# MAC-VO/MAC-VO

Measured on AMD Instinct MI355X. Metric: stereo frames/sec at 640x480 (hot path: cost volume + lookup, keypoint selection, covariance, PGO), higher is better.
Workload: dtype f32 via f16x2 (volume: fp32 operands row-scaled by powers of two and split into two fp16 pieces, three products, fp32 accumulate, scales undone exactly) + f32 (lookup/covariance) + f64 (PGO)

## Files before the change

### mac-vo_amd/csrc/frontend_ops.hip

```cpp
#include "common.h"
#include "randperm_dev.h"
#include "kp_draw_dev.h"
#include "match_cov_dev.h"
#include "pose_apply_dev.h"
#include "obs_filter_dev.h"
#include <math.h>

namespace {

__global__ __launch_bounds__(256) void frontend_epilogue_kernel(
    const float* __restrict__ flow, const float* __restrict__ logcov, int cov_is_log, int plane, float bl_fx,
    float bl_fx_sq, float* __restrict__ disparity, float* __restrict__ disparity_cov, float* __restrict__ depth,
    float* __restrict__ depth_cov, uint8_t* __restrict__ bad_mask, float* __restrict__ match_flow,
    float* __restrict__ match_cov) {
    MV_CHAIN_KERNEL_PRIO();
    const size_t lo = (size_t)blockIdx.y * plane;
    flow += 4 * lo; logcov += 4 * lo;
    if (disparity) disparity += lo;
    if (disparity_cov) disparity_cov += lo;
    if (depth) depth += lo;
    if (depth_cov) depth_cov += lo;
    if (bad_mask) bad_mask += lo;
    if (match_flow) match_flow += 2 * lo;
    if (match_cov) match_cov += 3 * lo;
// ... 12 lines not shown
    const size_t lo = (size_t)blockIdx.y * plane;
    flow += 4 * lo;
    if (D || M) logcov += 4 * lo;
    if (disparity) disparity += lo;
    if (D && disparity_cov) disparity_cov += lo;
    if (depth) depth += lo;
    if (D && depth_cov) depth_cov += lo;
    if (bad_mask) bad_mask += lo;
    if (match_flow) match_flow += 2 * lo;
    if (M && match_cov) match_cov += 3 * lo;
    const mvEpiArgs ea{flow, logcov, cov_is_log, bl_fx, bl_fx_sq, disparity, D ? disparity_cov : nullptr, depth, D ? depth_cov : nullptr, match_flow,
                       M ? match_cov : nullptr, bad_mask};
    for (int i = blockIdx.x * blockDim.x + threadIdx.x; i < plane; i += gridDim.x * blockDim.x) mv_epilogue_pixel_partial<D, M>(ea, plane, i);
}

__device__ __forceinline__ void kp_track_one(int n, int u0, int v0, const float* __restrict__ match_flow, const float* __restrict__ match_cov,
                                             const float* __restrict__ depth0, const float* __restrict__ disp0,
                                             const float* __restrict__ sdisp0, const float* __restrict__ sdd0,
                                             const float* __restrict__ depth1, const float* __restrict__ disp1,
                                             const float* __restrict__ sdisp1, const float* __restrict__ sdd1, int H, int W, int edge,
                                             float match_cov_default, float* __restrict__ out_kp0, float* __restrict__ out_kp1,
                                             uint8_t* __restrict__ out_inbound, float* __restrict__ out_vals, size_t vs,
                                             float* __restrict__ out_sigma0, float* __restrict__ out_sigma1) {
    const int plane = H * W;
    const bool ok0 = u0 >= 0 && u0 < W && v0 >= 0 && v0 < H;
    const int i0 = ok0 ? v0 * W + u0 : 0;
    const float u1 = (float)u0 + match_flow[i0];
    const float v1 = (float)v0 + match_flow[plane + i0];
    const bool inb = ok0 && (u1 < (float)(W - edge)) && (u1 > (float)edge) && (v1 < (float)(H - edge)) && (v1 > (float)edge);
    if (out_kp0) { out_kp0[2 * n] = (float)u0; out_kp0[2 * n + 1] = (float)v0; }
    out_kp1[2 * n] = u1;
    out_kp1[2 * n + 1] = v1;
    out_inbound[n] = inb;
    float* o = out_vals + n;
    o[0 * vs] = depth0[i0];
    o[1 * vs] = disp0 ? disp0[i0] : -1.f;
    o[2 * vs] = sdisp0 ? sdisp0[i0] : -1.f;
    o[3 * vs] = sdd0 ? sdd0[i0] : -1.f;
    if (inb) {
        const int i1 = (int)v1 * W + (int)u1;
        o[4 * vs] = depth1[i1];
        o[5 * vs] = disp1 ? disp1[i1] : -1.f;
        o[6 * vs] = sdisp1 ? sdisp1[i1] : -1.f;
        o[7 * vs] = sdd1 ? sdd1[i1] : -1.f;
    } else {
        o[4 * vs] = o[5 * vs] = o[6 * vs] = o[7 * vs] = 0.f;
    }
    const float suu = match_cov ? match_cov[i0] : -1.f;
    const float svv = match_cov ? match_cov[plane + i0] : -1.f;
    const float suv = match_cov ? match_cov[2 * plane + i0] : -1.f;
    o[8 * vs] = suu; o[9 * vs] = svv; o[10 * vs] = suv;
    if (out_sigma1) { out_sigma1[3 * n] = suu; out_sigma1[3 * n + 1] = svv; out_sigma1[3 * n + 2] = suv; }
    if (out_sigma0) { out_sigma0[3 * n] = match_cov_default; out_sigma0[3 * n + 1] = match_cov_default; out_sigma0[3 * n + 2] = 0.f; }
}

struct TrackArgs {
    const float *match_flow, *match_cov, *depth0, *disp0, *sdisp0, *sdd0, *depth1, *disp1, *sdisp1, *sdd1;
    int H, W, edge;
    float match_cov_default;
    float *out_kp0, *out_kp1;
    uint8_t* out_inbound;
    float *out_vals, *out_sigma0, *out_sigma1;
};
__device__ __forceinline__ void track_lane_offsets(TrackArgs& a, int lane, int N) {
    const size_t lp = (size_t)lane * a.H * a.W, ln = (size_t)lane * N;
    a.match_flow += 2 * lp;
    if (a.match_cov) a.match_cov += 3 * lp;
    a.depth0 += lp; a.depth1 += lp;
// ... 31 lines not shown
                                                       int64_t* __restrict__ out_uv, TrackArgs a, float fx, float fy, float cx, float cy,
                                                       float* __restrict__ pos_Tc) {
    const int n = blockIdx.x * blockDim.x + threadIdx.x;
    const int lane = blockIdx.y;
    if (n >= cnt.n[lane]) return;
    cand += (size_t)lane * cand_lane_stride;
    out_uv += 2 * (size_t)lane * cap;
    pos_Tc += 3 * (size_t)lane * cap;
    track_lane_offsets(a, lane, cap);
    const long pi = PERM_IN_ARGS ? (long)pa.idx[n] : (long)perm[(size_t)lane * cap + n];
    const int lin = cand[pi];
    const int u0 = lin % a.W, v0 = lin / a.W;
    out_uv[2 * n + 0] = u0;
    out_uv[2 * n + 1] = v0;
    const size_t vs = (size_t)gridDim.y * cap;
    kp_track_one(n, u0, v0, a.match_flow, a.match_cov, a.depth0, a.disp0, a.sdisp0, a.sdd0, a.depth1, a.disp1, a.sdisp1, a.sdd1, a.H,
                 a.W, a.edge, a.match_cov_default, a.out_kp0, a.out_kp1, a.out_inbound, a.out_vals, vs, a.out_sigma0, a.out_sigma1);
    const float u = (float)u0, v = (float)v0, d = a.out_vals[n];
    pos_Tc[3 * n] = d;
    pos_Tc[3 * n + 1] = ((u - cx) * d) / fx;
    pos_Tc[3 * n + 2] = ((v - cy) * d) / fy;
}

__global__ __launch_bounds__(256) void backproject_kernel(const float* __restrict__ kp_uv,
                                                          const float* __restrict__ depth_vals, int depth_stride,
                                                          float fx, float fy, float cx, float cy,
                                                          const float* __restrict__ pose, int cap, mvLaneCounts cnt,
                                                          size_t depth_lane_stride,
                                                          float* __restrict__ pos_Tc, float* __restrict__ pos_Tw,
                                                          double* __restrict__ rot) {
    const int n = blockIdx.x * blockDim.x + threadIdx.x;
    const int lane = blockIdx.y;
    const int N = cnt.n[lane];
// ... 123 lines not shown
    int32_t out[mvrp::MAX_HEAD];
};
template <int PM, int MODEL = MV_COV_MATCH, bool MODS = false, bool NOMATCH = false>
__global__ __launch_bounds__(256) void backend_front_kernel(const int32_t* __restrict__ cand, size_t cand_lane_stride, const int64_t* __restrict__ perm,
                                                            PermArg pa, int cap, mvLaneCounts cnt, int64_t* out_uv, TrackArgs a, float fx, float fy,
                                                            float cx, float cy, float* pos_Tc, const float* depth_map0, const float* depth_map1,
                                                            double* out_cov0, double* out_cov1, mvMatchCovParams cp, DrawArgs da) {
    __shared__ __attribute__((aligned(16))) char draw_raw[PM == 2 ? sizeof(DrawLds) : PM == 4 ? sizeof(mvkp::Scratch) : 16];
    DrawLds& D = *reinterpret_cast<DrawLds*>(draw_raw);
    const int lane = threadIdx.x & 63;
    const int n = blockIdx.x * 4 + (threadIdx.x >> 6);
    const int set = blockIdx.y, pl = blockIdx.z;
    int N;
    if constexpr (PM == 2) {
        const int64_t n_cand = da.count[(size_t)pl * da.count_stride];
        const bool adv = blockIdx.x == 0 && blockIdx.y == 0;
        N = mv_randperm_head_wg(da.state_in + (size_t)pl * mvrp::MT_STRIDE, adv ? da.state_out + (size_t)pl * mvrp::MT_STRIDE : nullptr, n_cand, da.k,
                                D.out, D.s, D.head);
        __syncthreads();
        if (adv) {
            for (int i = threadIdx.x; i < N; i += 256) da.out_perm[(size_t)pl * cap + i] = D.out[i];
            if (threadIdx.x == 0) { da.out_live[2 * pl] = N; da.out_live[2 * pl + 1] = (int32_t)n_cand; }
        }
    } else if constexpr (PM == 3) {
        if (da.count) {
            const int c = da.count[(size_t)pl * da.count_stride];
            N = c < 0 ? 0 : (c > cap ? cap : c);
        } else {
            N = cnt.n[pl];
        }
        if (da.out_live && blockIdx.x == 0 && blockIdx.y == 0 && threadIdx.x == 0) { da.out_live[2 * pl] = N; da.out_live[2 * pl + 1] = N; }
    } else if constexpr (PM == 4) {
        N = cnt.n[pl];
// ... 12 lines not shown
            u0 = lin % a.W;
            v0 = lin / a.W;
        } else if constexpr (PM == 3) {
            const int64_t* kp = perm + 2 * ((size_t)pl * cap + n);
            u0 = (int)kp[0];
            v0 = (int)kp[1];
        } else if constexpr (PM == 4) {
            mvkp::row_of(reinterpret_cast<mvkp::Scratch*>(draw_raw)->w, da.k, n, a.H, a.W, pa.idx[0], u0, v0);
        } else {
            mvkp::grid_row(mvkp::Grid{pa.idx[0], 0, pa.idx[1], pa.idx[2], pa.idx[3]}, n, u0, v0);
        }
        TrackArgs al = a;
        track_lane_offsets(al, pl, cap);
        const size_t ln = (size_t)pl * cap;
        float u, v, suu, svv, suv;
        if (set == 0) {
            if (lane == 0) {
                if (PM != 3 || out_uv != perm) {
                    out_uv[2 * (ln + n) + 0] = u0;
                    out_uv[2 * (ln + n) + 1] = v0;
                }
                kp_track_one(n, u0, v0, al.match_flow, al.match_cov, al.depth0, al.disp0, al.sdisp0, al.sdd0, al.depth1, al.disp1, al.sdisp1, al.sdd1,
                             al.H, al.W, al.edge, al.match_cov_default, al.out_kp0, al.out_kp1, al.out_inbound, al.out_vals, (size_t)gridDim.z * cap,
                             nullptr, nullptr);
                al.out_sigma0[3 * n + 2] = 0.f;
                const float uf = (float)u0, vf = (float)v0, d = al.out_vals[n];
                float* pt = pos_Tc + 3 * (ln + n);
                pt[0] = d;
                pt[1] = ((uf - cx) * d) / fx;
                pt[2] = ((vf - cy) * d) / fy;
            }
            u = (float)u0; v = (float)v0;
            suu = a.match_cov_default; svv = a.match_cov_default; suv = 0.f;
        } else {
            const int plane = al.H * al.W;
            const bool ok0 = u0 >= 0 && u0 < al.W && v0 >= 0 && v0 < al.H;
            const int i0 = ok0 ? v0 * al.W + u0 : 0;
            u = (float)u0 + al.match_flow[i0];
            v = (float)v0 + al.match_flow[plane + i0];
            if constexpr (NOMATCH) {
                if (lane == 0) { al.out_sigma1[3 * n] = -1.f; al.out_sigma1[3 * n + 1] = -1.f; al.out_sigma1[3 * n + 2] = -1.f; }
                const bool inb = ok0 && (u < (float)(al.W - al.edge)) && (u > (float)al.edge) && (v < (float)(al.H - al.edge)) && (v > (float)al.edge);
                const bool have_var = al.sdd1 != nullptr;
                const float var = have_var && inb ? al.sdd1[(int)v * al.W + (int)u] : 0.f;
                const mvcov::CovSet S1{depth_map1, nullptr, nullptr, nullptr, nullptr, out_cov1, nullptr, nullptr};
                mvcov::match_cov_wave_vals<MODEL, MODS, true>(S1, cp, cap, pl, n, u, v, da.nomatch_c, da.nomatch_c, 0.f, da.cov_mods, a.sdd1, var, have_var);
                return;
            }
            suu = al.match_cov ? al.match_cov[i0] : -1.f;
            svv = al.match_cov ? al.match_cov[plane + i0] : -1.f;
            suv = al.match_cov ? al.match_cov[2 * plane + i0] : -1.f;
            if (lane == 0) al.out_sigma1[3 * n + 2] = suv;
        }
        const mvcov::CovSet S{set ? depth_map1 : depth_map0, nullptr, set ? a.out_sigma1 : a.out_sigma0, nullptr, nullptr, set ? out_cov1 : out_cov0,
                              nullptr, nullptr};
        if constexpr (MODEL == MV_COV_MATCH && !MODS)
            mvcov::match_cov_wave_vals(S, cp, cap, pl, n, u, v, suu, svv, suv);
        else
            mvcov::match_cov_wave_vals<MODEL, MODS>(S, cp, cap, pl, n, u, v, suu, svv, suv, da.cov_mods, set ? a.sdd1 : a.sdd0);
    }
}

template <int PM, typename... Args>
void launch_backend_front(int model, int32_t mods, bool nomatch, float nomatch_c, dim3 grid, hipStream_t st, DrawArgs da, Args... args) {
    const bool m = mods != 0;
    da.cov_mods = mods;
    if constexpr (PM >= 3) if (nomatch) {
        da.nomatch_c = nomatch_c;
        if (model == MV_COV_MATCH && !m)
            hipLaunchKernelGGL((backend_front_kernel<PM, MV_COV_MATCH, false, true>), grid, dim3(256), 0, st, args..., da);
        else if (model == MV_COV_MATCH)
            hipLaunchKernelGGL((backend_front_kernel<PM, MV_COV_MATCH, true, true>), grid, dim3(256), 0, st, args..., da);
        else if (model == MV_COV_GMM && !m)
            hipLaunchKernelGGL((backend_front_kernel<PM, MV_COV_GMM, false, true>), grid, dim3(256), 0, st, args..., da);
// ... 355 lines not shown
```

### mac-vo_amd/csrc/kp_select.hip

```cpp
#include "common.h"
#include <math.h>

namespace {

#ifdef MV_KP_PROFILE
__device__ long long g_kp_stamps[16];
#define KP_STAMP(i) do { if (threadIdx.x == 0) g_kp_stamps[i] = wall_clock64(); } while (0)
#else
#define KP_STAMP(i)
#endif

constexpr int TILE_W = 64;
constexpr int TILE_H = 16;
constexpr int MAX_R = 7;
constexpr unsigned CAND_FLAG = 0x80000000u;

struct KpWs {
    unsigned long long* cand_bits;
    unsigned* rec_idx;
    float* rec_q;
    float* rec_d;
    int* counters;
    size_t lane_bytes;

// ... 341 lines not shown
                for (int j = 0; j < cb; ++j) {
                    const unsigned o = L.lst[j];
                    rank += (o < e) || (o == e && j < i);
                }
                if (rank == k) L.res = e;
            }
            __syncthreads();
            return key_float(L.res);
        }
        lo = nlo;
        hi = nhi;
        __syncthreads();
    }
}

template <int NT, bool FAST, int RPT, int WPT, bool USE_D>
__device__ __forceinline__ void kp_finish_body(const mvKpSelectParams& p, const KpWs& ws, int has_flow, int words_per_row,
                                               int32_t* __restrict__ out_cand, int32_t* __restrict__ out_count,
                                               float* __restrict__ out_stats, int n_rec, MedianLds& L,
                                               unsigned long long* lds_words) {
    constexpr int RD = USE_D ? RPT : 1;
    const int tid = threadIdx.x;
    const int H = p.H, W = p.W;
    const bool mapping = p.mode == MV_KP_MAPPING;
    const bool use_f = (p.mode == MV_KP_NODEPTH) || (p.mode == MV_KP_FULL && has_flow);
    const bool use_d = USE_D && (p.mode == MV_KP_FULL);
    const int n_words = H * words_per_row;

    unsigned kq[RPT], kd[RD], ridx[RPT];
    unsigned long long wreg[WPT];
    KP_STAMP(0);
    if (FAST) {
        const int cap = H * W;
#pragma unroll
        for (int r = 0; r < RPT; ++r) {
            const int i = min(r * NT + tid, cap - 1);
            ridx[r] = mapping ? 0u : ws.rec_idx[i];
            kq[r] = use_f ? __float_as_uint(ws.rec_q[i]) : 0u;
            if (USE_D) kd[r] = use_d ? __float_as_uint(ws.rec_d[i]) : 0u;
        }
#pragma unroll
        for (int j = 0; j < WPT; ++j) {
            const int w = j * NT + tid;
            wreg[j] = w < n_words ? ws.cand_bits[w] : 0ull;
        }
#pragma unroll
        for (int r = 0; r < RPT; ++r) {
            const bool live = r * NT + tid < n_rec;
            ridx[r] = live ? ridx[r] : 0u;
            kq[r] = live ? float_key(__uint_as_float(kq[r])) : NAN_KEY;
            if (USE_D) kd[r] = live ? float_key(__uint_as_float(kd[r])) : NAN_KEY;
        }
    }

    float med_f = NAN, thr_f = INFINITY, med_d = NAN, thr_d = INFINITY;
    KP_STAMP(1);
    if (use_f) {
        med_f = block_nanmedian<NT, FAST, RPT>(ws.rec_q, n_rec, kq, L);
        const float prod = med_f * 1.5f;
        thr_f = (prod < p.max_match_cov) ? prod : p.max_match_cov;
// ... 107 lines not shown
        out_stats[3] = thr_d;
    }
}

template <int NT, int RPT, int WPT, bool USE_D>
__global__ __launch_bounds__(NT) void kp_finish_kernel(mvKpSelectParams p, KpWs ws_all, int has_flow, int words_per_row,
                                                        int32_t* __restrict__ out_cand, int32_t* __restrict__ out_count,
                                                        float* __restrict__ out_stats) {
    __shared__ MedianLds L;
    extern __shared__ unsigned long long lds_words[];
    MV_CHAIN_KERNEL_PRIO();
    const KpWs ws = ws_all.lane(blockIdx.x);
    out_cand += (size_t)blockIdx.x * p.H * p.W;
    out_count += 4 * blockIdx.x;
    out_stats += 4 * blockIdx.x;
    const int n_rec = p.mode == MV_KP_MAPPING ? 0 : ws.counters[0];
    if (n_rec <= RPT * NT && p.H * words_per_row <= WPT * NT)
        kp_finish_body<NT, true, RPT, WPT, USE_D>(p, ws, has_flow, words_per_row, out_cand, out_count, out_stats, n_rec, L,
                                                  lds_words);
    else
        kp_finish_body<NT, false, RPT, WPT, USE_D>(p, ws, has_flow, words_per_row, out_cand, out_count, out_stats, n_rec, L,
                                                   lds_words);
}

template <int NT, int RPT, int WPT, bool USE_D>
static int launch_finish(const mvKpSelectParams& p, const KpWs& ws, int has_flow, int wpr, int32_t* out_cand,
                         int32_t* out_count, float* out_stats, int lanes, hipStream_t s) {
    const size_t dyn = (size_t)WPT * (NT / (WPT > 5 * 1024 / NT ? 8 : 2)) * sizeof(unsigned long long);
    hipLaunchKernelGGL((kp_finish_kernel<NT, RPT, WPT, USE_D>), dim3(lanes), dim3(NT), dyn, s, p, ws, has_flow, wpr, out_cand,
                       out_count, out_stats);
    return MV_OK;
}

__global__ __launch_bounds__(1024) void kp_map_scan_kernel(const unsigned long long* __restrict__ cand_bits, int n_words,
                                                            int* __restrict__ word_off, int32_t* __restrict__ out_count,
                                                            float* __restrict__ out_stats) {
    __shared__ int wave_tot[16];
// ... 189 lines not shown
```

### mac-vo_amd/csrc/match_cov_dev.h

```cpp
#pragma once
#include "common.h"
#include <math.h>

namespace mvcov {

constexpr int MAX_K = 31;
constexpr int MAX_TAPS_PER_LANE = (MAX_K * MAX_K + 63) / 64;

__device__ __forceinline__ float clamp_min_nanprop(float x, float m) { return (x < m) ? m : x; }

struct CovSet {
    const float* depth_map;
    const float* kp_uv;
    float* flow_cov;
    const float* depth_cov;
    const double* rot;
    double* out_cov;
    double* out_cov_rot;
    float* out_stats;
};

__device__ __forceinline__ void apply_modifiers(double c[9], int32_t mods) {
#pragma unroll
    for (int s = 0; s < 4; ++s) {
// ... 25 lines not shown
            for (int j = 0; j < 3; ++j)
                t[3 * i + j] = (R[3 * i] * c[j] + R[3 * i + 1] * c[3 + j]) + R[3 * i + 2] * c[6 + j];
        double* orot = out_cov_rot + (size_t)n * 9;
#pragma unroll
        for (int i = 0; i < 3; ++i)
#pragma unroll
            for (int j = 0; j < 3; ++j)
                orot[3 * i + j] = (t[3 * i] * R[3 * j] + t[3 * i + 1] * R[3 * j + 1]) + t[3 * i + 2] * R[3 * j + 2];
    }
    if (out_stats) {
        out_stats[2 * n] = mu;
        out_stats[2 * n + 1] = var;
    }
}

template <int MODEL = MV_COV_MATCH, bool MODS = false, bool NOMATCH = false>
__device__ __forceinline__ void match_cov_wave_vals(const CovSet& S, const mvMatchCovParams& p, int cap, int pl, int n, float u, float v,
                                                    float suu, float svv, float suv, int32_t mods = 0,
                                                    const float* depth_cov_map_all = nullptr ,
                                                    float var_given = 0.f, bool have_var = false ) {
    const int lane = threadIdx.x & 63;
    const size_t ln = (size_t)pl * cap;
    const float* __restrict__ depth_map = S.depth_map + (size_t)pl * p.H * p.W;
    float* __restrict__ flow_cov = S.flow_cov + 3 * ln;
    const float* __restrict__ depth_cov = S.depth_cov ? S.depth_cov + ln : nullptr;
    const double* __restrict__ rot = S.rot ? S.rot + 9 * pl : nullptr;
    double* __restrict__ out_cov = S.out_cov + 9 * ln;
    double* __restrict__ out_cov_rot = S.out_cov_rot ? S.out_cov_rot + 9 * ln : nullptr;
    float* __restrict__ out_stats = S.out_stats ? S.out_stats + 2 * ln : nullptr;

    if constexpr (MODEL == MV_COV_NONE) {
        if (lane == 0) {
            if constexpr (!NOMATCH) {
                flow_cov[3 * n] = suu;
                flow_cov[3 * n + 1] = svv;
            }
            double c[9] = {1.0, 0.0, 0.0, 0.0, 1.0, 0.0, 0.0, 0.0, 1.0};
            store_cov<MODS>(c, mods, rot, out_cov, out_cov_rot, out_stats, n, __builtin_nanf(""), __builtin_nanf(""));
        }
        return;
    }
    const float* __restrict__ depth_cov_map = MODEL == MV_COV_GMM ? depth_cov_map_all + (size_t)pl * p.H * p.W : nullptr;

    const int iu = (int)u, iv = (int)v;
    if constexpr (!NOMATCH) {
        suu = clamp_min_nanprop(suu, p.min_flow_cov_sq);
        svv = clamp_min_nanprop(svv, p.min_flow_cov_sq);
        if (lane == 0) {
            flow_cov[3 * n] = suu;
            flow_cov[3 * n + 1] = svv;
        }
    }
    bool patch_var;
    if constexpr (NOMATCH) patch_var = !have_var; else patch_var = p.use_patch_var;

    const float det = suu * svv - suv * suv;
    const float m00 = -0.5f * (svv / det), m01 = -0.5f * (-suv / det), m11 = -0.5f * (suu / det);
    const float cnorm = (2.f * 3.14159265358979323846f) * sqrtf(det);

    const int K = p.kernel_size, h = K >> 1, taps = K * K;
    float z[MAX_TAPS_PER_LANE], kv[MAX_TAPS_PER_LANE];
    float zc[MODEL == MV_COV_GMM ? MAX_TAPS_PER_LANE : 1];
    float ksum = 0.f;
#pragma unroll
    for (int r = 0; r < MAX_TAPS_PER_LANE; ++r) {
        const int idx = r * 64 + lane;
        z[r] = 0.f;
        kv[r] = 0.f;
        if constexpr (MODEL == MV_COV_GMM) zc[r] = 0.f;
        if (idx < taps) {
            const int a = idx / K, b = idx - a * K;
            int yy = iv + (a - h), xx = iu + (b - h);
            yy = min(max(yy, 0), p.H - 1);
            xx = min(max(xx, 0), p.W - 1);
            z[r] = depth_map[yy * p.W + xx];
            if constexpr (MODEL == MV_COV_GMM) zc[r] = depth_cov_map[yy * p.W + xx] + z[r] * z[r];
            const float x0 = (float)(a - h), x1 = (float)(b - h);
            const float q = (x0 * m00) * x0 + 2.f * ((x0 * m01) * x1) + (x1 * m11) * x1;
            kv[r] = expf(q) / cnorm;
            ksum += kv[r];
        }
    }
    ksum = wave_sum(ksum);

    float mu = 0.f, var;
    if constexpr (MODEL == MV_COV_GMM) {
        float psum = 0.f;
#pragma unroll
        for (int r = 0; r < MAX_TAPS_PER_LANE; ++r) {
            kv[r] = kv[r] / ksum;
            if (kv[r] < 1e-3f) kv[r] = 0.f;
            psum += kv[r];
        }
        psum = wave_sum(psum);
        float e2 = 0.f;
#pragma unroll
        for (int r = 0; r < MAX_TAPS_PER_LANE; ++r) {
            kv[r] = kv[r] / psum;
            mu += z[r] * kv[r];
            e2 += zc[r] * kv[r];
        }
        mu = wave_sum(mu);
        e2 = wave_sum(e2);
        if constexpr (NOMATCH) var = patch_var ? (e2 - mu * mu) / 2.f : var_given;
// ... 46 lines not shown
                    t[3 * i + j] = (R[3 * i] * c[j] + R[3 * i + 1] * c[3 + j]) + R[3 * i + 2] * c[6 + j];
            double* orot = out_cov_rot + (size_t)n * 9;
#pragma unroll
            for (int i = 0; i < 3; ++i)
#pragma unroll
                for (int j = 0; j < 3; ++j)
                    orot[3 * i + j] = (t[3 * i] * R[3 * j] + t[3 * i + 1] * R[3 * j + 1]) + t[3 * i + 2] * R[3 * j + 2];
        }
        if (out_stats) {
            out_stats[2 * n] = mu;
            out_stats[2 * n + 1] = var;
        }
    }
}


template <int MODEL = MV_COV_MATCH, bool MODS = false>
__device__ __forceinline__ void match_cov_wave(const CovSet& S, const mvMatchCovParams& p, int cap, int pl, int n, int32_t mods = 0,
                                               const float* depth_cov_map = nullptr) {
    const size_t ln = (size_t)pl * cap;
    const float* __restrict__ kp_uv = S.kp_uv + 2 * ln;
    const float* __restrict__ flow_cov = S.flow_cov + 3 * ln;
    match_cov_wave_vals<MODEL, MODS>(S, p, cap, pl, n, kp_uv[2 * n], kp_uv[2 * n + 1], flow_cov[3 * n], flow_cov[3 * n + 1], flow_cov[3 * n + 2],
                                     mods, depth_cov_map);
}

template <int MODEL, bool MODS>
__device__ __forceinline__ void match_cov_wave_nomatch(const CovSet& S, const mvMatchCovParams& p, int cap, int pl, int n, float c, int32_t mods,
                                                       const float* depth_cov_map) {
    const size_t ln = (size_t)pl * cap;
// ... 8 lines not shown
```

### mac-vo_amd/csrc/randperm.hip

```cpp
#include "common.h"
#include "randperm_dev.h"
#include <vector>

int mv_randperm_heads_emulated_state(uint32_t* state, const int64_t* n, int calls, int k, int threads, int64_t* out);

namespace {

__global__ __launch_bounds__(1024) void randperm_head_kernel(uint32_t* __restrict__ state, const int32_t* __restrict__ n_dev, int n_stride, int k, int cap,
                                                             int64_t* __restrict__ out, int32_t* __restrict__ n_sel, int nsel_stride) {
    __shared__ mvrp::Scratch s;
    __shared__ int32_t head[mvrp::NBUCKET];
    const int l = blockIdx.x;
    uint32_t* const st = state + (size_t)l * mvrp::MT_STRIDE;
    const int m = mv_randperm_head_wg(st, st, (int64_t)n_dev[(size_t)l * n_stride], k, out + (size_t)l * cap, s, head);
    if (threadIdx.x == 0) n_sel[(size_t)l * nsel_stride] = m;
}

}

extern "C" int mv_randperm_state_words(void) { return mvrp::MT_STRIDE; }
extern "C" int mv_randperm_max_head(void) { return mvrp::MAX_HEAD; }

extern "C" int mv_mt19937_seed(uint64_t seed, uint32_t* state_host) {
    MV_CHECK_ARG(state_host);
    mvrp::mt_seed((uint32_t)(seed & 0xffffffffull), state_host);
    return MV_OK;
}

extern "C" int mv_randperm_head_lanes(uint32_t* state, const int32_t* n_dev, int n_stride, int lanes, int k, int cap, int64_t* out_perm, int32_t* out_n_sel,
// ... 54 lines not shown
```

### mac-vo_amd/csrc/randperm_dev.h

```cpp
#pragma once
#include <stdint.h>

#if defined(__HIPCC__)
#define MV_RP_FN __host__ __device__ __forceinline__
#else
#define MV_RP_FN inline
#endif

namespace mvrp {

constexpr int MT_N = 624;
constexpr int MT_STRIDE = 640;
constexpr int MAX_HEAD = 512;
constexpr int NBUCKET = 1024;

struct Scratch {
    uint32_t mt[2][MT_N];
    int32_t t[MAX_HEAD], nxt[MAX_HEAD], ptr[MAX_HEAD], hit[MAX_HEAD];
};

MV_RP_FN uint32_t mt_f(uint32_t a, uint32_t b) {
    const uint32_t y = (a & 0x80000000u) | (b & 0x7fffffffu);
    return (y >> 1) ^ ((b & 1u) ? 0x9908b0dfu : 0u);
}
// ... 84 lines not shown
    while (s.ptr[i] >= 0) i = s.ptr[i];
    return i;
}

template <typename T>
MV_RP_FN void phase_emit(const Scratch& s, const Plan& pl, T* out, int tid, int nt) {
    for (int i = tid; i < pl.m; i += nt) {
        const int32_t h = s.hit[i];
        out[i] = (T)(h == -2 ? root_of(s, i) : (h >= 0 ? root_of(s, h) : s.t[i]));
    }
}

}

#if defined(__HIPCC__)
template <typename T>
__device__ __forceinline__ int mv_randperm_head_wg(const uint32_t* __restrict__ state_in, uint32_t* state_out, int64_t n, int k, T* out, mvrp::Scratch& s,
                                                   int32_t* head) {
    using namespace mvrp;
    const int tid = threadIdx.x, nt = blockDim.x;
    const Plan pl = plan_of(n, k);
    phase_clear(head, tid, nt);
    if (pl.advance > 0 || state_out) {
        for (int i = tid; i < MT_N; i += nt) s.mt[0][i] = state_in[i];
        int pos = (int)state_in[MT_N];
        __syncthreads();
        int cur = 0;
        int64_t produced = 0;
        const int64_t total = state_out ? pl.advance : (int64_t)pl.swaps;
        int64_t rem = total;
        while (rem > 0) {
            if (pos == MT_N) {
                phase_step(s.mt[cur], s.mt[cur ^ 1], tid, nt);
                __syncthreads();
                cur ^= 1;
                pos = 0;
            }
            const int take = (int)(rem < MT_N - pos ? rem : MT_N - pos);
            if (produced < pl.swaps) phase_draws(s.mt[cur], pos, take, produced, pl, s.t, tid, nt);
            pos += take;
// ... 1 lines not shown
            rem -= take;
        }
        if (state_out) {
            for (int i = tid; i < MT_N; i += nt) state_out[i] = s.mt[cur][i];
            if (tid == 0) state_out[MT_N] = (uint32_t)pos;
        }
    }
    __syncthreads();
    phase_insert(s, head, pl, tid, nt);
    __syncthreads();
    phase_link(s, head, pl, tid, nt);
    __syncthreads();
    phase_emit(s, pl, out, tid, nt);
    return pl.m;
}
#endif
```

Baseline: 7291.

## Hoist global loads ahead of dependent work in front and select kernels

Splits keypoint tracking into separate load, load-dependent and store phases so the tracker lane's gathers can be issued alongside the covariance window loads in the fused backend front kernel. The randperm state load is hoisted into registers before the draw, and the kp_finish preload of records and candidate bits is moved out of the body. The aim is to hide global-memory latency in small latency-bound kernels, at the cost of more live registers and possible occupancy pressure. A standalone timing probe script is also added.

```diff
diff --git a/mac-vo_amd/csrc/frontend_ops.hip b/mac-vo_amd/csrc/frontend_ops.hip
--- a/mac-vo_amd/csrc/frontend_ops.hip
+++ b/mac-vo_amd/csrc/frontend_ops.hip
@@ -50,44 +50,84 @@
     for (int i = blockIdx.x * blockDim.x + threadIdx.x; i < plane; i += gridDim.x * blockDim.x) mv_epilogue_pixel_partial<D, M>(ea, plane, i);
 }
 
-__device__ __forceinline__ void kp_track_one(int n, int u0, int v0, const float* __restrict__ match_flow, const float* __restrict__ match_cov,
-                                             const float* __restrict__ depth0, const float* __restrict__ disp0,
-                                             const float* __restrict__ sdisp0, const float* __restrict__ sdd0,
-                                             const float* __restrict__ depth1, const float* __restrict__ disp1,
-                                             const float* __restrict__ sdisp1, const float* __restrict__ sdd1, int H, int W, int edge,
-                                             float match_cov_default, float* __restrict__ out_kp0, float* __restrict__ out_kp1,
-                                             uint8_t* __restrict__ out_inbound, float* __restrict__ out_vals, size_t vs,
-                                             float* __restrict__ out_sigma0, float* __restrict__ out_sigma1) {
+struct KpTrackAt0 {
+    bool ok0;
+    float fu, fv, d0, p0, sp0, sd0, suu, svv, suv;
+};
+struct KpTrackAt1 {
+    float u1, v1;
+    bool inb;
+    float d1, p1, sp1, sd1;
+};
+__device__ __forceinline__ KpTrackAt0 kp_track_load0(int u0, int v0, const float* __restrict__ match_flow, const float* __restrict__ match_cov,
+                                                     const float* __restrict__ depth0, const float* __restrict__ disp0,
+                                                     const float* __restrict__ sdisp0, const float* __restrict__ sdd0, int H, int W) {
     const int plane = H * W;
-    const bool ok0 = u0 >= 0 && u0 < W && v0 >= 0 && v0 < H;
-    const int i0 = ok0 ? v0 * W + u0 : 0;
-    const float u1 = (float)u0 + match_flow[i0];
-    const float v1 = (float)v0 + match_flow[plane + i0];
-    const bool inb = ok0 && (u1 < (float)(W - edge)) && (u1 > (float)edge) && (v1 < (float)(H - edge)) && (v1 > (float)edge);
+    KpTrackAt0 t;
+    t.ok0 = u0 >= 0 && u0 < W && v0 >= 0 && v0 < H;
+    const int i0 = t.ok0 ? v0 * W + u0 : 0;
+    t.fu = match_flow[i0];
+    t.fv = match_flow[plane + i0];
+    t.d0 = depth0[i0];
+    t.p0 = disp0 ? disp0[i0] : -1.f;
+    t.sp0 = sdisp0 ? sdisp0[i0] : -1.f;
+    t.sd0 = sdd0 ? sdd0[i0] : -1.f;
+    t.suu = match_cov ? match_cov[i0] : -1.f;
+    t.svv = match_cov ? match_cov[plane + i0] : -1.f;
+    t.suv = match_cov ? match_cov[2 * plane + i0] : -1.f;
+    return t;
+}
+__device__ __forceinline__ KpTrackAt1 kp_track_load1(int u0, int v0, const KpTrackAt0& t0, const float* __restrict__ depth1,
+                                                     const float* __restrict__ disp1, const float* __restrict__ sdisp1,
+                                                     const float* __restrict__ sdd1, int H, int W, int edge) {
+    KpTrackAt1 t;
+    t.u1 = (float)u0 + t0.fu;
+    t.v1 = (float)v0 + t0.fv;
+    t.inb = t0.ok0 && (t.u1 < (float)(W - edge)) && (t.u1 > (float)edge) && (t.v1 < (float)(H - edge)) && (t.v1 > (float)edge);
+    if (t.inb) {
+        const int i1 = (int)t.v1 * W + (int)t.u1;
+        t.d1 = depth1[i1];
+        t.p1 = disp1 ? disp1[i1] : -1.f;
+        t.sp1 = sdisp1 ? sdisp1[i1] : -1.f;
+        t.sd1 = sdd1 ? sdd1[i1] : -1.f;
+    } else {
+        t.d1 = t.p1 = t.sp1 = t.sd1 = 0.f;
+    }
+    return t;
+}
+__device__ __forceinline__ void kp_track_store(int n, int u0, int v0, const KpTrackAt0& t0, const KpTrackAt1& t1, float match_cov_default,
+                                               float* __restrict__ out_kp0, float* __restrict__ out_kp1, uint8_t* __restrict__ out_inbound,
+                                               float* __restrict__ out_vals, size_t vs, float* __restrict__ out_sigma0,
+                                               float* __restrict__ out_sigma1) {
     if (out_kp0) { out_kp0[2 * n] = (float)u0; out_kp0[2 * n + 1] = (float)v0; }
-    out_kp1[2 * n] = u1;
-    out_kp1[2 * n + 1] = v1;
-    out_inbound[n] = inb;
+    out_kp1[2 * n] = t1.u1;
+    out_kp1[2 * n + 1] = t1.v1;
+    out_inbound[n] = t1.inb;
     float* o = out_vals + n;
-    o[0 * vs] = depth0[i0];
-    o[1 * vs] = disp0 ? disp0[i0] : -1.f;
-    o[2 * vs] = sdisp0 ? sdisp0[i0] : -1.f;
-    o[3 * vs] = sdd0 ? sdd0[i0] : -1.f;
-    if (inb) {
-        const int i1 = (int)v1 * W + (int)u1;
-        o[4 * vs] = depth1[i1];
-        o[5 * vs] = disp1 ? disp1[i1] : -1.f;
-        o[6 * vs] = sdisp1 ? sdisp1[i1] : -1.f;
-        o[7 * vs] = sdd1 ? sdd1[i1] : -1.f;
-    } else {
-        o[4 * vs] = o[5 * vs] = o[6 * vs] = o[7 * vs] = 0.f;
-    }
-    const float suu = match_cov ? match_cov[i0] : -1.f;
-    const float svv = match_cov ? match_cov[plane + i0] : -1.f;
-    const float suv = match_cov ? match_cov[2 * plane + i0] : -1.f;
-    o[8 * vs] = suu; o[9 * vs] = svv; o[10 * vs] = suv;
-    if (out_sigma1) { out_sigma1[3 * n] = suu; out_sigma1[3 * n + 1] = svv; out_sigma1[3 * n + 2] = suv; }
+    o[0 * vs] = t0.d0;
+    o[1 * vs] = t0.p0;
+    o[2 * vs] = t0.sp0;
+    o[3 * vs] = t0.sd0;
+    o[4 * vs] = t1.d1;
+    o[5 * vs] = t1.p1;
+    o[6 * vs] = t1.sp1;
+    o[7 * vs] = t1.sd1;
+    o[8 * vs] = t0.suu; o[9 * vs] = t0.svv; o[10 * vs] = t0.suv;
+    if (out_sigma1) { out_sigma1[3 * n] = t0.suu; out_sigma1[3 * n + 1] = t0.svv; out_sigma1[3 * n + 2] = t0.suv; }
     if (out_sigma0) { out_sigma0[3 * n] = match_cov_default; out_sigma0[3 * n + 1] = match_cov_default; out_sigma0[3 * n + 2] = 0.f; }
+}
+__device__ __forceinline__ float kp_track_one(int n, int u0, int v0, const float* __restrict__ match_flow, const float* __restrict__ match_cov,
+                                              const float* __restrict__ depth0, const float* __restrict__ disp0,
+                                              const float* __restrict__ sdisp0, const float* __restrict__ sdd0,
+                                              const float* __restrict__ depth1, const float* __restrict__ disp1,
+                                              const float* __restrict__ sdisp1, const float* __restrict__ sdd1, int H, int W, int edge,
+                                              float match_cov_default, float* __restrict__ out_kp0, float* __restrict__ out_kp1,
+                                              uint8_t* __restrict__ out_inbound, float* __restrict__ out_vals, size_t vs,
+                                              float* __restrict__ out_sigma0, float* __restrict__ out_sigma1) {
+    const KpTrackAt0 t0 = kp_track_load0(u0, v0, match_flow, match_cov, depth0, disp0, sdisp0, sdd0, H, W);
+    const KpTrackAt1 t1 = kp_track_load1(u0, v0, t0, depth1, disp1, sdisp1, sdd1, H, W, edge);
+    kp_track_store(n, u0, v0, t0, t1, match_cov_default, out_kp0, out_kp1, out_inbound, out_vals, vs, out_sigma0, out_sigma1);
+    return t0.d0;
 }
 
 struct TrackArgs {
@@ -149,9 +189,9 @@
     out_uv[2 * n + 0] = u0;
     out_uv[2 * n + 1] = v0;
     const size_t vs = (size_t)gridDim.y * cap;
-    kp_track_one(n, u0, v0, a.match_flow, a.match_cov, a.depth0, a.disp0, a.sdisp0, a.sdd0, a.depth1, a.disp1, a.sdisp1, a.sdd1, a.H,
-                 a.W, a.edge, a.match_cov_default, a.out_kp0, a.out_kp1, a.out_inbound, a.out_vals, vs, a.out_sigma0, a.out_sigma1);
-    const float u = (float)u0, v = (float)v0, d = a.out_vals[n];
+    const float d = kp_track_one(n, u0, v0, a.match_flow, a.match_cov, a.depth0, a.disp0, a.sdisp0, a.sdd0, a.depth1, a.disp1, a.sdisp1, a.sdd1, a.H,
+                                 a.W, a.edge, a.match_cov_default, a.out_kp0, a.out_kp1, a.out_inbound, a.out_vals, vs, a.out_sigma0, a.out_sigma1);
+    const float u = (float)u0, v = (float)v0;
     pos_Tc[3 * n] = d;
     pos_Tc[3 * n + 1] = ((u - cx) * d) / fx;
     pos_Tc[3 * n + 2] = ((v - cy) * d) / fy;
@@ -305,9 +345,9 @@
     int N;
     if constexpr (PM == 2) {
         const int64_t n_cand = da.count[(size_t)pl * da.count_stride];
+        const mvRandpermStateRegs<256> st = mv_randperm_state_load<256>(da.state_in + (size_t)pl * mvrp::MT_STRIDE);
         const bool adv = blockIdx.x == 0 && blockIdx.y == 0;
-        N = mv_randperm_head_wg(da.state_in + (size_t)pl * mvrp::MT_STRIDE, adv ? da.state_out + (size_t)pl * mvrp::MT_STRIDE : nullptr, n_cand, da.k,
-                                D.out, D.s, D.head);
+        N = mv_randperm_head_draw<256>(st, adv ? da.state_out + (size_t)pl * mvrp::MT_STRIDE : nullptr, n_cand, da.k, D.out, D.s, D.head);
         __syncthreads();
         if (adv) {
             for (int i = threadIdx.x; i < N; i += 256) da.out_perm[(size_t)pl * cap + i] = D.out[i];
@@ -350,50 +390,61 @@
         track_lane_offsets(al, pl, cap);
         const size_t ln = (size_t)pl * cap;
         float u, v, suu, svv, suv;
+        float z[mvcov::MAX_TAPS_PER_LANE], kv[mvcov::MAX_TAPS_PER_LANE], zc[mvcov::cov_zc_slots(MODEL)], ksum = 0.f;
+        int ta[mvcov::MAX_TAPS_PER_LANE];
+        const bool tracker = set == 0 && lane == 0;
+        KpTrackAt0 t0{};
+        KpTrackAt1 t1{};
         if (set == 0) {
-            if (lane == 0) {
-                if (PM != 3 || out_uv != perm) {
-                    out_uv[2 * (ln + n) + 0] = u0;
-                    out_uv[2 * (ln + n) + 1] = v0;
-                }
-                kp_track_one(n, u0, v0, al.match_flow, al.match_cov, al.depth0, al.disp0, al.sdisp0, al.sdd0, al.depth1, al.disp1, al.sdisp1, al.sdd1,
-                             al.H, al.W, al.edge, al.match_cov_default, al.out_kp0, al.out_kp1, al.out_inbound, al.out_vals, (size_t)gridDim.z * cap,
-                             nullptr, nullptr);
-                al.out_sigma0[3 * n + 2] = 0.f;
-                const float uf = (float)u0, vf = (float)v0, d = al.out_vals[n];
-                float* pt = pos_Tc + 3 * (ln + n);
-                pt[0] = d;
-                pt[1] = ((uf - cx) * d) / fx;
-                pt[2] = ((vf - cy) * d) / fy;
-            }
             u = (float)u0; v = (float)v0;
             suu = a.match_cov_default; svv = a.match_cov_default; suv = 0.f;
+            mvcov::cov_window_load<MODEL>(depth_map0, a.sdd0, cp, pl, u, v, z, zc, ta);
+            if (lane == 0) t0 = kp_track_load0(u0, v0, al.match_flow, al.match_cov, al.depth0, al.disp0, al.sdisp0, al.sdd0, al.H, al.W);
         } else {
             const int plane = al.H * al.W;
             const bool ok0 = u0 >= 0 && u0 < al.W && v0 >= 0 && v0 < al.H;
             const int i0 = ok0 ? v0 * al.W + u0 : 0;
-            u = (float)u0 + al.match_flow[i0];
-            v = (float)v0 + al.match_flow[plane + i0];
+            const float fu = al.match_flow[i0], fv = al.match_flow[plane + i0];
+            if constexpr (!NOMATCH) {
+                suu = al.match_cov ? al.match_cov[i0] : -1.f;
+                svv = al.match_cov ? al.match_cov[plane + i0] : -1.f;
+                suv = al.match_cov ? al.match_cov[2 * plane + i0] : -1.f;
+            }
+            u = (float)u0 + fu;
+            v = (float)v0 + fv;
+            mvcov::cov_window_load<MODEL>(depth_map1, a.sdd1, cp, pl, u, v, z, zc, ta);
             if constexpr (NOMATCH) {
                 if (lane == 0) { al.out_sigma1[3 * n] = -1.f; al.out_sigma1[3 * n + 1] = -1.f; al.out_sigma1[3 * n + 2] = -1.f; }
                 const bool inb = ok0 && (u < (float)(al.W - al.edge)) && (u > (float)al.edge) && (v < (float)(al.H - al.edge)) && (v > (float)al.edge);
                 const bool have_var = al.sdd1 != nullptr;
                 const float var = have_var && inb ? al.sdd1[(int)v * al.W + (int)u] : 0.f;
                 const mvcov::CovSet S1{depth_map1, nullptr, nullptr, nullptr, nullptr, out_cov1, nullptr, nullptr};
-                mvcov::match_cov_wave_vals<MODEL, MODS, true>(S1, cp, cap, pl, n, u, v, da.nomatch_c, da.nomatch_c, 0.f, da.cov_mods, a.sdd1, var, have_var);
+                suu = da.nomatch_c; svv = da.nomatch_c; suv = 0.f;
+                mvcov::cov_wave_weights<MODEL, true>(nullptr, cp, n, suu, svv, suv, ta, kv, ksum);
+                mvcov::cov_wave_finish<MODEL, MODS, true>(S1, cp, cap, pl, n, u, v, suu, svv, suv, da.cov_mods, z, zc, kv, ksum, var, have_var);
                 return;
             }
-            suu = al.match_cov ? al.match_cov[i0] : -1.f;
-            svv = al.match_cov ? al.match_cov[plane + i0] : -1.f;
-            suv = al.match_cov ? al.match_cov[2 * plane + i0] : -1.f;
             if (lane == 0) al.out_sigma1[3 * n + 2] = suv;
         }
         const mvcov::CovSet S{set ? depth_map1 : depth_map0, nullptr, set ? a.out_sigma1 : a.out_sigma0, nullptr, nullptr, set ? out_cov1 : out_cov0,
                               nullptr, nullptr};
-        if constexpr (MODEL == MV_COV_MATCH && !MODS)
-            mvcov::match_cov_wave_vals(S, cp, cap, pl, n, u, v, suu, svv, suv);
-        else
-            mvcov::match_cov_wave_vals<MODEL, MODS>(S, cp, cap, pl, n, u, v, suu, svv, suv, da.cov_mods, set ? a.sdd1 : a.sdd0);
+        mvcov::cov_wave_weights<MODEL, false>(S.flow_cov + 3 * ln, cp, n, suu, svv, suv, ta, kv, ksum);
+        if (tracker) t1 = kp_track_load1(u0, v0, t0, al.depth1, al.disp1, al.sdisp1, al.sdd1, al.H, al.W, al.edge);
+        mvcov::cov_wave_finish<MODEL, MODS, false>(S, cp, cap, pl, n, u, v, suu, svv, suv, da.cov_mods, z, zc, kv, ksum, 0.f, false);
+        if (tracker) {
+            if (PM != 3 || out_uv != perm) {
+                out_uv[2 * (ln + n) + 0] = u0;
+                out_uv[2 * (ln + n) + 1] = v0;
+            }
+            kp_track_store(n, u0, v0, t0, t1, al.match_cov_default, al.out_kp0, al.out_kp1, al.out_inbound, al.out_vals, (size_t)gridDim.z * cap, nullptr,
+                           nullptr);
+            al.out_sigma0[3 * n + 2] = 0.f;
+            const float uf = (float)u0, vf = (float)v0, d = t0.d0;
+            float* pt = pos_Tc + 3 * (ln + n);
+            pt[0] = d;
+            pt[1] = ((uf - cx) * d) / fx;
+            pt[2] = ((vf - cy) * d) / fy;
+        }
     }
 }
 
diff --git a/mac-vo_amd/csrc/kp_select.hip b/mac-vo_amd/csrc/kp_select.hip
--- a/mac-vo_amd/csrc/kp_select.hip
+++ b/mac-vo_amd/csrc/kp_select.hip
@@ -379,11 +379,36 @@
     }
 }
 
+template <int NT, int RPT, int WPT, bool USE_D>
+__device__ __forceinline__ void kp_finish_preload(const mvKpSelectParams& p, const KpWs& ws, int has_flow, int words_per_row,
+                                                  unsigned (&kq)[RPT], unsigned (&kd)[USE_D ? RPT : 1], unsigned (&ridx)[RPT],
+                                                  unsigned long long (&wreg)[WPT]) {
+    const int tid = threadIdx.x;
+    const bool mapping = p.mode == MV_KP_MAPPING;
+    const bool use_f = (p.mode == MV_KP_NODEPTH) || (p.mode == MV_KP_FULL && has_flow);
+    const bool use_d = USE_D && (p.mode == MV_KP_FULL);
+    const int n_words = p.H * words_per_row;
+    const int cap = p.H * p.W;
+#pragma unroll
+    for (int r = 0; r < RPT; ++r) {
+        const int i = min(r * NT + tid, cap - 1);
+        ridx[r] = mapping ? 0u : ws.rec_idx[i];
+        kq[r] = use_f ? __float_as_uint(ws.rec_q[i]) : 0u;
+        if (USE_D) kd[r] = use_d ? __float_as_uint(ws.rec_d[i]) : 0u;
+    }
+#pragma unroll
+    for (int j = 0; j < WPT; ++j) {
+        const int w = j * NT + tid;
+        wreg[j] = w < n_words ? ws.cand_bits[w] : 0ull;
+    }
+}
+
 template <int NT, bool FAST, int RPT, int WPT, bool USE_D>
 __device__ __forceinline__ void kp_finish_body(const mvKpSelectParams& p, const KpWs& ws, int has_flow, int words_per_row,
                                                int32_t* __restrict__ out_cand, int32_t* __restrict__ out_count,
                                                float* __restrict__ out_stats, int n_rec, MedianLds& L,
-                                               unsigned long long* lds_words) {
+                                               unsigned long long* lds_words, unsigned (&kq)[RPT], unsigned (&kd)[USE_D ? RPT : 1],
+                                               unsigned (&ridx)[RPT], unsigned long long (&wreg)[WPT]) {
     constexpr int RD = USE_D ? RPT : 1;
     const int tid = threadIdx.x;
     const int H = p.H, W = p.W;
@@ -392,23 +417,8 @@
     const bool use_d = USE_D && (p.mode == MV_KP_FULL);
     const int n_words = H * words_per_row;
 
-    unsigned kq[RPT], kd[RD], ridx[RPT];
-    unsigned long long wreg[WPT];
     KP_STAMP(0);
     if (FAST) {
-        const int cap = H * W;
-#pragma unroll
-        for (int r = 0; r < RPT; ++r) {
-            const int i = min(r * NT + tid, cap - 1);
-            ridx[r] = mapping ? 0u : ws.rec_idx[i];
-            kq[r] = use_f ? __float_as_uint(ws.rec_q[i]) : 0u;
-            if (USE_D) kd[r] = use_d ? __float_as_uint(ws.rec_d[i]) : 0u;
-        }
-#pragma unroll
-        for (int j = 0; j < WPT; ++j) {
-            const int w = j * NT + tid;
-            wreg[j] = w < n_words ? ws.cand_bits[w] : 0ull;
-        }
 #pragma unroll
         for (int r = 0; r < RPT; ++r) {
             const bool live = r * NT + tid < n_rec;
@@ -546,13 +556,17 @@
     out_cand += (size_t)blockIdx.x * p.H * p.W;
     out_count += 4 * blockIdx.x;
     out_stats += 4 * blockIdx.x;
+    unsigned kq[RPT], kd[USE_D ? RPT : 1], ridx[RPT];
+    unsigned long long wreg[WPT];
+    const bool fits = p.H * words_per_row <= WPT * NT;
+    if (fits) kp_finish_preload<NT, RPT, WPT, USE_D>(p, ws, has_flow, words_per_row, kq, kd, ridx, wreg);
     const int n_rec = p.mode == MV_KP_MAPPING ? 0 : ws.counters[0];
-    if (n_rec <= RPT * NT && p.H * words_per_row <= WPT * NT)
+    if (n_rec <= RPT * NT && fits)
         kp_finish_body<NT, true, RPT, WPT, USE_D>(p, ws, has_flow, words_per_row, out_cand, out_count, out_stats, n_rec, L,
-                                                  lds_words);
+                                                  lds_words, kq, kd, ridx, wreg);
     else
         kp_finish_body<NT, false, RPT, WPT, USE_D>(p, ws, has_flow, words_per_row, out_cand, out_count, out_stats, n_rec, L,
-                                                   lds_words);
+                                                   lds_words, kq, kd, ridx, wreg);
 }
 
 template <int NT, int RPT, int WPT, bool USE_D>
diff --git a/mac-vo_amd/csrc/match_cov_dev.h b/mac-vo_amd/csrc/match_cov_dev.h
--- a/mac-vo_amd/csrc/match_cov_dev.h
+++ b/mac-vo_amd/csrc/match_cov_dev.h
@@ -63,14 +63,79 @@
     }
 }
 
+constexpr int cov_zc_slots(int model) { return model == MV_COV_GMM ? MAX_TAPS_PER_LANE : 1; }
+
+template <int MODEL>
+__device__ __forceinline__ void cov_window_load(const float* depth_map_all, const float* depth_cov_map_all ,
+                                                const mvMatchCovParams& p, int pl, float u, float v, float (&z)[MAX_TAPS_PER_LANE],
+                                                float (&zc)[cov_zc_slots(MODEL)], int (&ta)[MAX_TAPS_PER_LANE]) {
+    if constexpr (MODEL == MV_COV_NONE) return;
+    const int lane = threadIdx.x & 63;
+    const float* __restrict__ depth_map = depth_map_all + (size_t)pl * p.H * p.W;
+    const float* __restrict__ depth_cov_map = MODEL == MV_COV_GMM ? depth_cov_map_all + (size_t)pl * p.H * p.W : nullptr;
+    const int iu = (int)u, iv = (int)v;
+    const int K = p.kernel_size, h = K >> 1, taps = K * K;
+#pragma unroll
+    for (int r = 0; r < MAX_TAPS_PER_LANE; ++r) {
+        const int idx = r * 64 + lane;
+        float zr = 0.f, cr = 0.f;
+        int ar = 0;
+        if (idx < taps) {
+            const int a = idx / K, b = idx - a * K;
+            ar = a;
+            int yy = iv + (a - h), xx = iu + (b - h);
+            yy = min(max(yy, 0), p.H - 1);
+            xx = min(max(xx, 0), p.W - 1);
+            zr = depth_map[yy * p.W + xx];
+            if constexpr (MODEL == MV_COV_GMM) cr = depth_cov_map[yy * p.W + xx];
+        }
+        z[r] = zr;
+        ta[r] = ar;
+        if constexpr (MODEL == MV_COV_GMM) zc[r] = cr;
+    }
+}
+
+template <int MODEL, bool NOMATCH>
+__device__ __forceinline__ void cov_wave_weights(float* __restrict__ flow_cov , const mvMatchCovParams& p, int n, float& suu,
+                                                 float& svv, float suv, const int (&ta)[MAX_TAPS_PER_LANE], float (&kv)[MAX_TAPS_PER_LANE], float& ksum) {
+    if constexpr (MODEL == MV_COV_NONE) return;
+    const int lane = threadIdx.x & 63;
+    if constexpr (!NOMATCH) {
+        suu = clamp_min_nanprop(suu, p.min_flow_cov_sq);
+        svv = clamp_min_nanprop(svv, p.min_flow_cov_sq);
+        if (lane == 0) {
+            flow_cov[3 * n] = suu;
+            flow_cov[3 * n + 1] = svv;
+        }
+    }
+    const float det = suu * svv - suv * suv;
+    const float m00 = -0.5f * (svv / det), m01 = -0.5f * (-suv / det), m11 = -0.5f * (suu / det);
+    const float cnorm = (2.f * 3.14159265358979323846f) * sqrtf(det);
+
+    const int K = p.kernel_size, h = K >> 1, taps = K * K;
+    ksum = 0.f;
+#pragma unroll
+    for (int r = 0; r < MAX_TAPS_PER_LANE; ++r) {
+        const int idx = r * 64 + lane;
+        float kr = 0.f;
+        if (idx < taps) {
+            const int a = ta[r], b = idx - a * K;
+            const float x0 = (float)(a - h), x1 = (float)(b - h);
+            const float q = (x0 * m00) * x0 + 2.f * ((x0 * m01) * x1) + (x1 * m11) * x1;
+            kr = expf(q) / cnorm;
+            ksum += kr;
+        }
+        kv[r] = kr;
+    }
+    ksum = wave_sum(ksum);
+}
+
 template <int MODEL = MV_COV_MATCH, bool MODS = false, bool NOMATCH = false>
-__device__ __forceinline__ void match_cov_wave_vals(const CovSet& S, const mvMatchCovParams& p, int cap, int pl, int n, float u, float v,
-                                                    float suu, float svv, float suv, int32_t mods = 0,
-                                                    const float* depth_cov_map_all = nullptr ,
-                                                    float var_given = 0.f, bool have_var = false ) {
+__device__ __forceinline__ void cov_wave_finish(const CovSet& S, const mvMatchCovParams& p, int cap, int pl, int n, float u, float v, float suu, float svv,
+                                                float suv, int32_t mods, float (&z)[MAX_TAPS_PER_LANE], float (&zc)[cov_zc_slots(MODEL)],
+                                                float (&kv)[MAX_TAPS_PER_LANE], float ksum, float var_given, bool have_var) {
     const int lane = threadIdx.x & 63;
     const size_t ln = (size_t)pl * cap;
-    const float* __restrict__ depth_map = S.depth_map + (size_t)pl * p.H * p.W;
     float* __restrict__ flow_cov = S.flow_cov + 3 * ln;
     const float* __restrict__ depth_cov = S.depth_cov ? S.depth_cov + ln : nullptr;
     const double* __restrict__ rot = S.rot ? S.rot + 9 * pl : nullptr;
@@ -89,54 +154,15 @@
         }
         return;
     }
-    const float* __restrict__ depth_cov_map = MODEL == MV_COV_GMM ? depth_cov_map_all + (size_t)pl * p.H * p.W : nullptr;
-
-    const int iu = (int)u, iv = (int)v;
-    if constexpr (!NOMATCH) {
-        suu = clamp_min_nanprop(suu, p.min_flow_cov_sq);
-        svv = clamp_min_nanprop(svv, p.min_flow_cov_sq);
-        if (lane == 0) {
-            flow_cov[3 * n] = suu;
-            flow_cov[3 * n + 1] = svv;
-        }
-    }
     bool patch_var;
     if constexpr (NOMATCH) patch_var = !have_var; else patch_var = p.use_patch_var;
-
-    const float det = suu * svv - suv * suv;
-    const float m00 = -0.5f * (svv / det), m01 = -0.5f * (-suv / det), m11 = -0.5f * (suu / det);
-    const float cnorm = (2.f * 3.14159265358979323846f) * sqrtf(det);
-
-    const int K = p.kernel_size, h = K >> 1, taps = K * K;
-    float z[MAX_TAPS_PER_LANE], kv[MAX_TAPS_PER_LANE];
-    float zc[MODEL == MV_COV_GMM ? MAX_TAPS_PER_LANE : 1];
-    float ksum = 0.f;
-#pragma unroll
-    for (int r = 0; r < MAX_TAPS_PER_LANE; ++r) {
-        const int idx = r * 64 + lane;
-        z[r] = 0.f;
-        kv[r] = 0.f;
-        if constexpr (MODEL == MV_COV_GMM) zc[r] = 0.f;
-        if (idx < taps) {
-            const int a = idx / K, b = idx - a * K;
-            int yy = iv + (a - h), xx = iu + (b - h);
-            yy = min(max(yy, 0), p.H - 1);
-            xx = min(max(xx, 0), p.W - 1);
-            z[r] = depth_map[yy * p.W + xx];
-            if constexpr (MODEL == MV_COV_GMM) zc[r] = depth_cov_map[yy * p.W + xx] + z[r] * z[r];
-            const float x0 = (float)(a - h), x1 = (float)(b - h);
-            const float q = (x0 * m00) * x0 + 2.f * ((x0 * m01) * x1) + (x1 * m11) * x1;
-            kv[r] = expf(q) / cnorm;
-            ksum += kv[r];
-        }
-    }
-    ksum = wave_sum(ksum);
 
     float mu = 0.f, var;
     if constexpr (MODEL == MV_COV_GMM) {
         float psum = 0.f;
 #pragma unroll
         for (int r = 0; r < MAX_TAPS_PER_LANE; ++r) {
+            zc[r] = zc[r] + z[r] * z[r];
             kv[r] = kv[r] / ksum;
             if (kv[r] < 1e-3f) kv[r] = 0.f;
             psum += kv[r];
@@ -213,6 +239,17 @@
     }
 }
 
+template <int MODEL = MV_COV_MATCH, bool MODS = false, bool NOMATCH = false>
+__device__ __forceinline__ void match_cov_wave_vals(const CovSet& S, const mvMatchCovParams& p, int cap, int pl, int n, float u, float v,
+                                                    float suu, float svv, float suv, int32_t mods = 0,
+                                                    const float* depth_cov_map_all = nullptr ,
+                                                    float var_given = 0.f, bool have_var = false ) {
+    float z[MAX_TAPS_PER_LANE], kv[MAX_TAPS_PER_LANE], zc[cov_zc_slots(MODEL)], ksum = 0.f;
+    int ta[MAX_TAPS_PER_LANE];
+    cov_window_load<MODEL>(S.depth_map, depth_cov_map_all, p, pl, u, v, z, zc, ta);
+    cov_wave_weights<MODEL, NOMATCH>(S.flow_cov + 3 * (size_t)pl * cap, p, n, suu, svv, suv, ta, kv, ksum);
+    cov_wave_finish<MODEL, MODS, NOMATCH>(S, p, cap, pl, n, u, v, suu, svv, suv, mods, z, zc, kv, ksum, var_given, have_var);
+}
 
 template <int MODEL = MV_COV_MATCH, bool MODS = false>
 __device__ __forceinline__ void match_cov_wave(const CovSet& S, const mvMatchCovParams& p, int cap, int pl, int n, int32_t mods = 0,
diff --git a/mac-vo_amd/csrc/randperm.hip b/mac-vo_amd/csrc/randperm.hip
--- a/mac-vo_amd/csrc/randperm.hip
+++ b/mac-vo_amd/csrc/randperm.hip
@@ -12,7 +12,7 @@
     __shared__ int32_t head[mvrp::NBUCKET];
     const int l = blockIdx.x;
     uint32_t* const st = state + (size_t)l * mvrp::MT_STRIDE;
-    const int m = mv_randperm_head_wg(st, st, (int64_t)n_dev[(size_t)l * n_stride], k, out + (size_t)l * cap, s, head);
+    const int m = mv_randperm_head_wg<1024>(st, st, (int64_t)n_dev[(size_t)l * n_stride], k, out + (size_t)l * cap, s, head);
     if (threadIdx.x == 0) n_sel[(size_t)l * nsel_stride] = m;
 }
 
diff --git a/mac-vo_amd/csrc/randperm_dev.h b/mac-vo_amd/csrc/randperm_dev.h
--- a/mac-vo_amd/csrc/randperm_dev.h
+++ b/mac-vo_amd/csrc/randperm_dev.h
@@ -122,16 +122,38 @@
 }
 
 #if defined(__HIPCC__)
-template <typename T>
-__device__ __forceinline__ int mv_randperm_head_wg(const uint32_t* __restrict__ state_in, uint32_t* state_out, int64_t n, int k, T* out, mvrp::Scratch& s,
-                                                   int32_t* head) {
+template <int NT>
+struct mvRandpermStateRegs {
+    uint32_t w[(mvrp::MT_N + NT - 1) / NT];
+    uint32_t pos;
+};
+template <int NT>
+__device__ __forceinline__ mvRandpermStateRegs<NT> mv_randperm_state_load(const uint32_t* __restrict__ state_in) {
+    mvRandpermStateRegs<NT> r;
+    const int tid = threadIdx.x;
+#pragma unroll
+    for (int j = 0; j < (mvrp::MT_N + NT - 1) / NT; ++j) {
+        const int i = j * NT + tid;
+        r.w[j] = state_in[i < mvrp::MT_N ? i : mvrp::MT_N - 1];
+    }
+    r.pos = state_in[mvrp::MT_N];
+    return r;
+}
+
+template <int NT, typename T>
+__device__ __forceinline__ int mv_randperm_head_draw(const mvRandpermStateRegs<NT>& pre, uint32_t* state_out, int64_t n, int k, T* out, mvrp::Scratch& s,
+                                                     int32_t* head) {
     using namespace mvrp;
-    const int tid = threadIdx.x, nt = blockDim.x;
+    const int tid = threadIdx.x, nt = NT;
     const Plan pl = plan_of(n, k);
     phase_clear(head, tid, nt);
     if (pl.advance > 0 || state_out) {
-        for (int i = tid; i < MT_N; i += nt) s.mt[0][i] = state_in[i];
-        int pos = (int)state_in[MT_N];
+#pragma unroll
+        for (int j = 0; j < (MT_N + NT - 1) / NT; ++j) {
+            const int i = j * NT + tid;
+            if (i < MT_N) s.mt[0][i] = pre.w[j];
+        }
+        int pos = (int)pre.pos;
         __syncthreads();
         int cur = 0;
         int64_t produced = 0;
@@ -163,4 +185,10 @@
     phase_emit(s, pl, out, tid, nt);
     return pl.m;
 }
+
+template <int NT, typename T>
+__device__ __forceinline__ int mv_randperm_head_wg(const uint32_t* __restrict__ state_in, uint32_t* state_out, int64_t n, int k, T* out, mvrp::Scratch& s,
+                                                   int32_t* head) {
+    return mv_randperm_head_draw<NT>(mv_randperm_state_load<NT>(state_in), state_out, n, k, out, s, head);
+}
 #endif
diff --git a/profiles/probes/front_finish_alone.py b/profiles/probes/front_finish_alone.py
--- /dev/null
+++ b/profiles/probes/front_finish_alone.py
@@ -0,0 +1,84 @@
+#!/usr/bin/env python
+import argparse
+import ctypes as C
+import os
+import statistics
+import sys
+
+sys.path.insert(0, os.path.dirname(os.path.dirname(os.path.dirname(os.path.abspath(__file__)))))
+import torch
+
+from macvo_amd import _lib as L
+from macvo_amd import ops
+
+
+def period(fn, reps, rounds):
+    for _ in range(20):
+        fn()
+    torch.cuda.synchronize()
+    out = []
+    for _ in range(rounds):
+        e0, e1 = torch.cuda.Event(enable_timing=True), torch.cuda.Event(enable_timing=True)
+        e0.record()
+        for _ in range(reps):
+            fn()
+        e1.record()
+        torch.cuda.synchronize()
+        out.append(e0.elapsed_time(e1) * 1e3 / reps)
+    return statistics.median(out), min(out), max(out)
+
+
+def main():
+    ap = argparse.ArgumentParser()
+    ap.add_argument("--reps", type=int, default=400)
+    ap.add_argument("--rounds", type=int, default=5)
+    a = ap.parse_args()
+    dev = torch.device("cuda:0")
+    lib = L.load()
+    print("library:", os.environ.get("MACVO_HIP_LIB") or L.LIB_PATH)
+    g = torch.Generator().manual_seed(0)
+    H, W, k, cap, n_cand, mw = 480, 640, 200, 256, 3000, 32
+    mk = lambda c, lo, hi: (lo + (hi - lo) * torch.rand(c, H, W, generator=g)).to(dev)
+    flow, cov = (torch.randn(2, H, W, generator=g) * 3).to(dev), mk(3, 0.1, 2.0)
+    maps = [mk(1, 2, 40) for _ in range(8)]
+    vv, uu = torch.meshgrid(torch.arange(mw, H - mw), torch.arange(mw, W - mw), indexing="ij")
+    interior = (vv * W + uu).reshape(-1)
+    cand = torch.zeros(H * W, dtype=torch.int32)
+    cand[:n_cand] = interior[torch.randperm(interior.numel(), generator=g)[:n_cand]].sort().values.int()
+    cand = cand.to(dev)
+    count = torch.tensor([n_cand, 0, 0, 0], dtype=torch.int32, device=dev)
+    st_in = ops.mt19937_state([5], dev)
+    st_out = torch.zeros_like(st_in)
+    i64 = lambda *s: torch.zeros(s, dtype=torch.int64, device=dev)
+    f32 = lambda *s: torch.zeros(s, dtype=torch.float32, device=dev)
+    perm, live, kp0_uv = i64(cap), torch.zeros(2, dtype=torch.int32, device=dev), i64(cap, 2)
+    kp0, kp1, inb, vals = f32(cap, 2), f32(cap, 2), torch.zeros(cap, dtype=torch.uint8, device=dev), f32(11, cap)
+    s0, s1, pos = f32(cap, 3), f32(cap, 3), f32(cap, 3)
+    c0, c1 = torch.zeros(cap, 9, dtype=torch.float64, device=dev), torch.zeros(cap, 9, dtype=torch.float64, device=dev)
+    p = L.mvMatchCovParams(H, W, 31, 1, 320.0, 320.0, 320.0, 240.0, 0.25 ** 2, 0.05)
+    s = ops._stream()
+    fargs = (cand.data_ptr(), H * W, count.data_ptr(), 4, st_in.data_ptr(), st_out.data_ptr(), k, 1, cap, flow.data_ptr(), cov.data_ptr(),
+             *[m.data_ptr() for m in maps], mw, 0.25, C.byref(p), perm.data_ptr(), live.data_ptr(), kp0_uv.data_ptr(), kp0.data_ptr(), kp1.data_ptr(),
+             inb.data_ptr(), vals.data_ptr(), s0.data_ptr(), s1.data_ptr(), pos.data_ptr(), c0.data_ptr(), c1.data_ptr(), s)
+    assert lib.mv_backend_front_draw_lanes(*fargs) == 0
+    med, lo, hi = period(lambda: lib.mv_backend_front_draw_lanes(*fargs), a.reps, a.rounds)
+    print(f"mv_backend_front_draw_lanes (backend_front_kernel<2>, {k} of {n_cand} candidates, 31 x 31)  {med:7.2f} us  [{lo:.2f} .. {hi:.2f}]")
+    print("live rows / candidates of the last call:", live.tolist())
+
+    fc = torch.exp(torch.randn(1, 3, H, W, generator=g)).to(dev)
+    fc[:, 2] = 0
+    sp = L.mvKpSelectParams(H, W, L.MV_KP_NODEPTH, 7, mw, 0.0, 0.0, 100.0)
+    nbytes = lib.mv_kp_select_workspace_bytes(H, W)
+    ws = torch.zeros((nbytes + 7) // 8, dtype=torch.int64, device=dev)
+    out_cand = torch.empty(H * W, dtype=torch.int32, device=dev)
+    cnt, stats = torch.empty(4, dtype=torch.int32, device=dev), torch.empty(4, device=dev)
+    uargs = (fc.data_ptr(), None, None, None, None, None, None, C.byref(sp), ws.data_ptr(), ws.numel() * 8, out_cand.data_ptr(), cnt.data_ptr(),
+             stats.data_ptr(), 1, s)
+    assert lib.mv_kp_select_lanes(*uargs) == 0
+    med, lo, hi = period(lambda: lib.mv_kp_select_lanes(*uargs), a.reps, a.rounds)
+    print(f"mv_kp_select_lanes (kp_nms_kernel<false> + kp_finish_kernel<1024, 16, 5>)               {med:7.2f} us  [{lo:.2f} .. {hi:.2f}]")
+    print("records / candidates of the last call:", int(cnt[1]), int(cnt[0]))
+
+
+if __name__ == "__main__":
+    main()
```

Result: no change. 7342 (median of 2 runs) (+0.7%).
